# control-toolbox/CTDirect.jl

Hardware: AMD Instinct MI355X
Metric: NLP callback evals/s (constraints+sparse Jac), N-step Goddard, 1/2/4/8 GPU (higher is better)
Workload: dtype f64

## Files before the change

ctdirect.jl_amd/csrc/ctd_engine.hip:

```cpp
#include <hip/hip_runtime.h>
#include <hip/hiprtc.h>
#include <dlfcn.h>

#include <cstdio>
#include <functional>
#include <map>
#include <mutex>
#include <cstdlib>
#include <cstring>
#include <memory>
#include <new>
#include <string>
#include <vector>

#include "../../include/ctdirect_hip.h"
#include "ctd_host.hpp"
#include "ctd_kernels.hpp"
#include "ctd_hess_kernels.hpp"
#include "ctd_hess_step.hpp"
#include "ctd_iter_kernels.hpp"
#include "ctd_prod_kernels.hpp"
#include "ctd_hprod_kernels.hpp"
#include "ctd_kkt_kernels.hpp"
#include "ctd_diag_kernels.hpp"
// ... 383 lines not shown
    if (blocks > 0x7fffffff) return fail(h, CTD_EINVAL, std::string(c.fn()) + ": grid too large");
    pp.nblocks = (int32_t)blocks;
    const int32_t st = partial.grow(h, blocks * kMaxNV, c.fn());
    if (st) return st;
    pp.partial = partial.p;
    hipError_t e = hipErrorInvalidValue;
    if (h->rt) {
        const JitModule& jm = h->jit[c.op.fam][c.shard()];
        void* args[] = {&a, &x_dev};
        e = jit_launch(jm.f[c.op.f0], (int)blocks, 256, 0, h->stream, args);
        if (e == hipSuccess) e = jit_launch(jm.f[c.op.f0 + 1], 1, 64, 0, h->stream, args);
    }
    for_problem(h->model.problem, [&](auto tag) {
        using P = typename decltype(tag)::type;
        e = c.shard() ? launch_prod_units<P, K, true>(a, x_dev, h->stream) : launch_prod_units<P, K, false>(a, x_dev, h->stream);
    });
    return c.launched(h, e);
}

extern "C" {

const char* ctd_strerror(int32_t st) {
    switch (st) {
        case CTD_OK: return "ok";
        case CTD_EINVAL: return "invalid argument";
        case CTD_EGRID: return "given time grid is not strictly increasing";
        case CTD_ESCHEME: return "unknown discretization method";
        case CTD_EPATTERN: return "sparsity pattern not available";
        case CTD_EPROBLEM: return "problem not in the compiled registry";
        case CTD_ENODEVICE: return "no HIP device bound to this handle (there is no CPU fallback)";
        case CTD_EHIP: return "HIP runtime error";
        case CTD_ENOMEM: return "out of memory";
        default: return "unknown status";
    }
}

const char* ctd_last_error(const ctd_handle* h) { return h ? h->err.c_str() : g_create_err.c_str(); }

int32_t ctd_create(const ctd_desc* desc, ctd_handle** out) {
    if (!desc || !out) return fail(nullptr, CTD_EINVAL, "ctd_create: null argument");
    *out = nullptr;
    struct Del { void operator()(ctd_handle* p) const { if (p) destroy_handle(p); } };
    std::unique_ptr<ctd_handle, Del> h(new (std::nothrow) ctd_handle());
    if (!h) return fail(nullptr, CTD_ENOMEM, "ctd_create: out of memory");
    HostDesc hd{desc->problem, desc->scheme, desc->pattern_mode, desc->grid_size, desc->time_grid, desc->time_grid_len,
                desc->control_steps > 1 ? desc->control_steps : 1, desc->value_order};
    if (desc->reserved0 != 0) return fail(nullptr, CTD_EINVAL, "ctd_create: ctd_desc.reserved0 must be 0 (zero-initialise the descriptor: memset / ctd_desc d = {0})");
    std::string err;
    int st;
    try {
        st = build_model(hd, h->model, err);
    } catch (const std::bad_alloc&) {
        return fail(nullptr, CTD_ENOMEM, "ctd_create: out of memory while building the model");
    }
    if (st) return fail(nullptr, st, err);
    const Model& mo = h->model;
    if (!runtime_ocp(mo.problem)) {
        const char* bad = nullptr;
        for_problem(mo.problem, [&](auto tag) {
            using P = typename decltype(tag)::type;
            for_scheme<true>(mo.L, [&](auto t) { bad = static_layout_mismatch<P, t.sc, t.s>(mo.L); });
        });
        if (bad) return fail(nullptr, CTD_EINVAL, std::string("ctd_create: the static layout of the kernel instantiation differs from the model's layout in field '") + bad + "'");
        if (mo.pattern_mode == 0 && mo.order == 0) {
            for_problem(mo.problem, [&](auto tag) {
                using P = typename decltype(tag)::type;
                for_scheme<true>(mo.L, [&](auto t) { bad = static_emit_mismatch<P, t.sc, t.s>(mo.L, mo.Lseg, mo.vr); });
            });
            if (bad) return fail(nullptr, CTD_EINVAL, std::string("ctd_create: the static emit geometry of the kernel instantiation differs from the model's in '") + bad + "'");
        }
    }
    if (mo.L.cs > 3 && desc->device >= 0 && !runtime_ocp(mo.problem))
        return fail(nullptr, CTD_EINVAL, "ctd_create: control_steps > 3 needs an OCP registered at run time (ctd_register_ocp); the compiled registry holds the midpoint kernels for 1, 2 and 3 controls per step");
    h->step_begin = desc->step_begin;
    h->step_end = desc->step_end;
    if (h->step_begin == 0 && h->step_end == 0) h->step_end = mo.L.N;
    if (h->step_begin < 0 || h->step_end > mo.L.N || h->step_begin >= h->step_end)
        return fail(nullptr, CTD_EINVAL, "ctd_create: shard [step_begin, step_end) is not inside [0, N)");
    h->tile = env_int("CTD_TILE", 0);
    h->lean_ok = env_int("CTD_LEAN", 1) ? 1 : 0;
    if (h->lean_ok && env_int("CTD_STATIC_EMIT", 1) && !runtime_ocp(mo.problem) && mo.pattern_mode == 0 && mo.order == 0 &&
        h->step_begin == 0 && h->step_end == mo.L.N)
        h->lean_ok |= 2;
    if (h->tile <= 0) h->tile = default_tile(mo, h->step_end - h->step_begin);
    int maxb = 256;
    for_problem(mo.problem, [&](auto tag) { maxb = decltype(tag)::type::MAXB; });
    h->rt = runtime_ocp(mo.problem);
    if (h->rt) maxb = h->rt->maxb;
    h->block = env_int("CTD_BLOCK", 0);
    if (h->block <= 0) {
        h->block = 256;
        const int64_t ntl = (h->step_end - h->step_begin + h->tile - 1) / h->tile;
        if (ntl <= 512 && mo.nch_dyn <= 1 && mo.Lseg > 0 && 320 / mo.Lseg > 256 / mo.Lseg && mo.Lseg * (320 / mo.Lseg) * 10 >= 320 * 9) h->block = 320;
    }
    if (h->block < 64 || (h->block % 64)) h->block = 256;
    if (h->block > maxb) h->block = maxb;
    mo.fill_kparams(h->kp, h->step_begin, h->step_end, h->tile);
    h->lds_bytes = (size_t)lds_doubles(h->kp) * sizeof(double);
    const int debug_stop = env_int("CTD_DEBUG_STOP", 0);
    const size_t lds_cap = h->rt ? 64 * 1024 : 80 * 1024;
    while (h->lds_bytes > lds_cap && h->tile > 1) {
        h->tile = (h->tile + 1) / 2;
        mo.fill_kparams(h->kp, h->step_begin, h->step_end, h->tile);
        h->lds_bytes = (size_t)lds_doubles(h->kp) * sizeof(double);
    }
    const bool long_mid = mo.L.sc == SC_MIDPOINT && mo.L.cs == 1;
    if (desc->device >= 0 && !h->rt && env_int("CTD_TILE", 0) <= 0 && mo.nch_dyn <= 1 && (mo.L.sc == SC_IRK || long_mid) && h->tile >= 16) {
        DeviceGuard dgq(desc->device);
        if (dgq.err == hipSuccess) {
            auto resident = [&](int tile, size_t& lds) {
                KParams kq;
                mo.fill_kparams(kq, h->step_begin, h->step_end, tile);
                lds = (size_t)lds_doubles(kq) * sizeof(double);
                int r = 0;
                for_problem(mo.problem, [&](auto tag) { r = occupancy_cons_jac<typename decltype(tag)::type>(kq, h->block, lds); });
                (void)hipGetLastError();
                return r;
            };
            size_t l0 = 0;
            const int r0 = resident(h->tile, l0);
            const int64_t ns = h->step_end - h->step_begin, cap = 256 * (int64_t)r0;
            if (r0 > 0 && (ns + h->tile - 1) / h->tile >= env_int("CTD_LONG_GRID_ROUNDS", 8) * cap && maxb >= 512 && env_int("CTD_BLOCK", 0) <= 0 &&
                env_int("CTD_LONG_GRID", 1)) {
                int tbest = h->tile;
                for (int tt = h->tile + 1; tt <= 256; ++tt) {
                    KParams kq;
                    mo.fill_kparams(kq, h->step_begin, h->step_end, tt);
                    if ((size_t)lds_doubles(kq) * sizeof(double) > (long_mid ? 74u : 64u) * 1024) break;
                    tbest = tt;
                }
                if (tbest > h->tile) {
                    h->tile = tbest;
                    h->block = 512;
                    mo.fill_kparams(h->kp, h->step_begin, h->step_end, h->tile);
                    h->lds_bytes = (size_t)lds_doubles(h->kp) * sizeof(double);
                }
            } else if (mo.L.sc == SC_IRK && r0 > 0 && (ns + h->tile - 1) / h->tile > cap) {
                int tmax = 48;
                for (; tmax > h->tile; --tmax) { size_t l = 0; if (resident(tmax, l) >= r0 && l <= lds_cap) break; }
                const int64_t rounds = (ns + (int64_t)tmax * cap - 1) / ((int64_t)tmax * cap);
                const int64_t tb = (ns + rounds * cap - 1) / (rounds * cap);
                if (tb > h->tile && tb <= tmax) {
                    h->tile = (int)tb;
                    mo.fill_kparams(h->kp, h->step_begin, h->step_end, h->tile);
                    h->lds_bytes = (size_t)lds_doubles(h->kp) * sizeof(double);
                }
            }
        }
    }
    h->grid = h->kp.ntiles + h->kp.has_edge;
    h->kp.debug_stop = debug_stop;
    h->out_mb = 8.0 * ((double)(h->step_end - h->step_begin) * (mo.L.cb + mo.Lseg + (double)mo.L.nv * mo.vr)) / 1.0e6;
    h->kp.wt_store = h->out_mb <= kWtMB ? 1 : 0;
    if (const int wt = env_int("CTD_WT_STORE", -1); wt >= 0) h->kp.wt_store = wt ? 1 : 0;
    h->device = desc->device;
    if (h->device >= 0) {
        int ndev = 0;
        if (hipGetDeviceCount(&ndev) != hipSuccess || h->device >= ndev)
            return fail(nullptr, CTD_ENODEVICE, "ctd_create: HIP device not available");
        ctd_handle* hp = h.get();
        if (h->lds_bytes > 160 * 1024) return fail(nullptr, CTD_EINVAL, "ctd_create: tile does not fit the 160 KiB LDS");
        DeviceGuard dg_(hp->device); HIP_TRY(nullptr, dg_.err);
        if (desc->stream_mode == CTD_STREAM_GIVEN) { hp->stream = (hipStream_t)desc->stream; hp->own_stream = false; }
        else { HIP_TRY(nullptr, hipStreamCreateWithFlags(&hp->stream, hipStreamNonBlocking)); hp->own_stream = true; }
        HIP_TRY(nullptr, upload(hp->d_tau, mo.tau));
        HIP_TRY(nullptr, upload(hp->d_tmpl, mo.tmpl));
// ... 1740 lines not shown
```

ctdirect.jl_amd/csrc/ctd_kernel_body.hpp:

```cpp
#pragma once
#include "ctd_layout.hpp"


namespace ctd {

#if defined(CTD_SUBSTAMPS) && defined(__HIP_DEVICE_COMPILE__)
#ifndef CTD_SUB_WAVE0
#define CTD_SUB_WAVE0 0
#endif
#define CTD_SUB(kp, id)                                                                                              \
    do {                                                                                                             \
        __builtin_amdgcn_sched_barrier(0);                                                                           \
        __builtin_amdgcn_s_waitcnt(0);                                                                               \
        if ((kp).stamps && (threadIdx.x & 63) == 0 && threadIdx.x >= 64 * CTD_SUB_WAVE0 && threadIdx.x < 64 * CTD_SUB_WAVE0 + 128) \
            (kp).stamps[(size_t)gridDim.x * 12 + ((size_t)blockIdx.x * 2 + (threadIdx.x >> 6) - CTD_SUB_WAVE0) * 8 + (id)] = clock64(); \
        __builtin_amdgcn_sched_barrier(0);                                                                           \
    } while (0)
#else
#define CTD_SUB(kp, id) do { } while (0)
#endif
#if defined(CTD_SUBSTAMPS_EMIT) && defined(__HIP_DEVICE_COMPILE__)
#define CTD_SUBE(kp, id)                                                                                             \
    do {                                                                                                             \
        __builtin_amdgcn_sched_barrier(0);                                                                           \
// ... 1522 lines not shown
                        for (int u = 0; u < 4; ++u) {
                            const int s = s0 + u * par;
                            if (s < nreg) emit_store(&out[s * Ls + k], a[u] * b[u] + beta, kp.wt_store);
                        }
                    }
                }
            } else {
                uint32_t code = (hp && tid < Ls) ? pre_->b : (tid < Ls ? cx.codes[tid] : 0u);
                int q = 0;
                for (int k = tid; k < Ls; k += nthr, ++q) {
                    uint32_t nxt = 0u;
                    bool have = false;
                    if constexpr (NB > 1) {
                        if (hp && q < NB - 1) {
                            have = true;
#pragma unroll
                            for (int e = 0; e < NB - 1; ++e)
                                if (e == q) nxt = pre_->more[e];
                        }
                    }
                    if (!have) nxt = k + nthr < Ls ? cx.codes[k + nthr] : 0u;
                    const int bt = code_beta(code);
                    const double beta = bt == 0 ? 0.0 : (bt == 1 ? 1.0 : -1.0);
                    const double* pc = cx.rec + (sl0 - code_crec(code)) * stride + R.oC + code_ci(code);
                    const double* pd = cx.rec + (sl0 - code_drec(code)) * stride + code_di(code);
                    const int last = nreg - 1;
                    for (int s0 = 0; s0 < nreg; s0 += 4) {
                        double a[4], b[4];
#pragma unroll
                        for (int u = 0; u < 4; ++u) {
                            const int s = s0 + u < last ? s0 + u : last;
                            a[u] = pc[s * stride];
                            b[u] = pd[s * stride];
                        }
#pragma unroll
                        for (int u = 0; u < 4; ++u)
                            if (s0 + u < nreg) emit_store(&out[(s0 + u) * Ls + k], a[u] * b[u] + beta, kp.wt_store);
                    }
                    code = nxt;
                }
            }
        }
    }
    CTD_SUBE(kp, 2);
    if (kp.vr > 0) {
        const int vr = kp.vr;
        const int par = (int)fast_div((uint32_t)nthr, kp.div_vr);
#pragma unroll
        for (int kk = 0; kk < P::NV; ++kk) {
            double* out = out_vals<B>(kp, bl) + kp.vcol_base[kk] + cx.a * (int64_t)vr;
            const uint32_t* codes = cx.vcodes + kk * vr;
            if (par >= 1) {
                if (tid < par * vr) {
                    const int g = (int)fast_div((uint32_t)tid, kp.div_vr), k = tid - g * vr;
                    const uint32_t code = hp ? pre_->v[kk] : codes[k];
                    const double* pc = cx.rec + (slot0 + g) * stride + R.oC + code_ci(code);
                    const double* pd = cx.rec + (slot0 + g) * stride + code_di(code);
                    const int adv = par * stride;
                    if (LEAN || k >= kp.vr_early)
                        for (int s = g; s < nsteps; s += par, pc += adv, pd += adv) emit_store(&out[s * vr + k], (*pc) * (*pd), kp.wt_store);
                }
            } else {
                for (int k = tid; k < vr; k += nthr) {
                    const uint32_t code = codes[k];
                    const double* pc = cx.rec + slot0 * stride + R.oC + code_ci(code);
                    const double* pd = cx.rec + slot0 * stride + code_di(code);
                    for (int s = 0; s < nsteps; ++s, pc += stride, pd += stride) emit_store(&out[s * vr + k], (*pc) * (*pd), kp.wt_store);
                }
            }
        }
    }
    CTD_SUBE(kp, 3);
}
template <class P, int SC, int S, int NB = 1, bool B = false, bool LEAN = false>
CTD_HD void phase_emit(const KParams& kp, const BlockCtx& cx, int tid, int nthr, const EmitPreT<NB>* pre = nullptr,
                       const BatchLd bl = BatchLd{}) {
    if (pre != nullptr) phase_emit_impl<P, SC, S, NB, B, LEAN>(kp, cx, tid, nthr, *pre, pre->have != 0, bl);
    else phase_emit_impl<P, SC, S, NB, B, LEAN>(kp, cx, tid, nthr, EmitPreT<NB>{}, false, bl);
}

}

#include "ctd_emit_static.hpp"

#if !defined(__HIPCC_RTC__)
#include "ctd_problems.hpp"
#include "ctd_sym_registry.hpp"
#endif
```

ctdirect.jl_amd/csrc/ctd_kernels.hpp:

```cpp
#pragma once
#if !defined(__HIPCC_RTC__)
#include <hip/hip_runtime.h>
#include <hip/hip_ext.h>
#endif

#include "ctd_kernel_body.hpp"
#if !defined(__HIPCC_RTC__)
#include "ctd_problems.hpp"
#endif

namespace ctd {

#ifndef CTD_MULTI_TILE_LOOP
#define CTD_MULTI_TILE_LOOP 0
#endif
constexpr bool kMultiTileLoop = CTD_MULTI_TILE_LOOP != 0;

template <bool DBG>
__device__ __forceinline__ void ctd_stamp(const KParams& kp, int slot) {
    if constexpr (DBG) {
        if (kp.stamps && threadIdx.x == 0) {
            unsigned long long* p = kp.stamps + ((size_t)blockIdx.x * 6 + slot) * 2;
            p[0] = wall_clock64();
            p[1] = clock64();
// ... 42 lines not shown
template <class P, int SC, int S, bool DBG, bool B = false, bool LEAN = false>
__device__ __forceinline__ void cons_jac_body(const KParams& kp, const double* __restrict__ xu, int block, double* ctd_lds,
                                              const BatchLd bl = BatchLd{}) {
    if constexpr (B) xu += batch_member() * bl.ldx;
    ctd_pin_kernargs<SC == SC_IRK ? S : 0, LEAN>(kp, xu);
    ctd_stamp<DBG>(kp, 0);
    if (DBG && kp.debug_stop == 1) return;
    const int tid = (int)threadIdx.x, nthr = (int)blockDim.x;
    if constexpr (DirectTile<P, SC>::value) {
        const BlockCtx cx = make_direct_ctx<LEAN>(kp, block, ctd_lds, xu, LV<P, SC, S, LEAN>::blk(kp), LEAN ? P::NV : -1);
        const EmitPre pre = emit_prefetch<P, 1, LEAN>(kp, cx, tid, nthr);
        ctd_stamp<DBG>(kp, 1);
        phase_eval<P, SC, S, RegEval<P, SC, S>::value, 1, B, LEAN>(kp, cx, tid, nthr, &pre, bl);
        ctd_pin_emit_kernargs<LEAN>(kp);
        __syncthreads();
        ctd_stamp<DBG>(kp, 2);
        ctd_stamp<DBG>(kp, 3);
        if (DBG && kp.debug_stop >= 2 && kp.debug_stop <= 4) return;
        phase_emit<P, SC, S, 1, B, LEAN>(kp, cx, tid, nthr, &pre, bl);
        ctd_stamp<DBG>(kp, 4);
        if (DBG && kp.stamps) {
            __builtin_amdgcn_s_waitcnt(0);
            __syncthreads();
            ctd_stamp<DBG>(kp, 5);
        }
        return;
    }
    BlockCtx cx = make_ctx<LEAN>(kp, block, ctd_lds);
    constexpr int NB = EmitN<P, SC, S>::value;
    EmitPreT<NB> pre = {};
    const bool use_pre = !cx.is_edge && !codes_staged(kp);
    if (use_pre) pre = emit_prefetch<P, NB, LEAN>(kp, cx, tid, nthr);
    phase_load<P, SC, S, true, LEAN>(kp, cx, xu, tid, nthr);
    const int nblk = kp.ntiles + kp.has_edge;
    for (;;) {
        __syncthreads();
        ctd_stamp<DBG>(kp, 1);
        if (DBG && kp.debug_stop == 2) return;
        phase_eval<P, SC, S, false, 1, B, LEAN>(kp, cx, tid, nthr, nullptr, bl);
        ctd_pin_emit_kernargs<LEAN>(kp);
        __syncthreads();
        ctd_stamp<DBG>(kp, 2);
        if (DBG && kp.debug_stop == 3) return;
        if (!Dirs<P>::FUSED && !fin_folded<P, SC, S>(cx)) {
            phase_fin<P, SC, S>(kp, cx, tid, nthr);
            __syncthreads();
        }
        if (SC == SC_TRAPEZE) {
            phase_fin2<P, SC, S>(kp, cx, tid, nthr);
            __syncthreads();
        }
        ctd_stamp<DBG>(kp, 3);
        if (DBG && kp.debug_stop == 4) return;
        block += kp.wg_stride;
        const bool more = kMultiTileLoop && kp.wg_stride > 0 && !cx.is_edge && block < nblk;
        BlockCtx nx = cx;
        TileIn tin{0.0, 0.0, 0.0};
        if (more) {
            nx = make_ctx<LEAN>(kp, block, ctd_lds);
            tin = load_issue<P>(kp, nx, xu, tid, nthr);
        }
        phase_emit_impl<P, SC, S, NB, B, LEAN>(kp, cx, tid, nthr, pre, use_pre, bl);
        ctd_stamp<DBG>(kp, 4);
        if (!more) break;
        load_commit<P, SC, S>(kp, nx, xu, tin, tid, nthr);
        cx = nx;
    }
    if (DBG && kp.stamps) {
        __builtin_amdgcn_s_waitcnt(0);
        __syncthreads();
        ctd_stamp<DBG>(kp, 5);
    }
}

template <class P, int SC, int S> struct MinWaves {
    static constexpr int value = (P::NX <= 12 && !(SC == SC_MIDPOINT && S > 1)) ? 4 : 1;
};

template <class P, int SC, int S, bool DBG, bool LEAN = false>
__global__ void __launch_bounds__(P::MAXB, (MinWaves<P, SC, S>::value)) cons_jac_kernel(const KParams kp, const double* __restrict__ xu) {
    extern __shared__ double ctd_lds[];
    cons_jac_body<P, SC, S, DBG, false, LEAN>(kp, xu, (int)blockIdx.x, ctd_lds);
}
template <class P, int SC, int S, bool DBG, int NTHR, bool WT>
__device__ __forceinline__ void cons_jac_static_body(const KParams& kp, const double* __restrict__ xu, int block, double* ctd_lds) {
    if (__builtin_expect(block < kp.has_edge, 0)) {
        cons_jac_body<P, SC, S, DBG, false, true>(kp, xu, block, ctd_lds);
        return;
    }
#if defined(__HIP_DEVICE_COMPILE__)
    asm volatile("" ::"s"(kp.has_edge), "s"(kp.T), "s"(kp.HL), "s"(kp.HH), "s"(kp.step_begin), "s"(kp.step_end), "s"(kp.L.N),
                 "s"(kp.L.v_off), "s"(kp.L.stagewise), "s"(kp.L.euler), "s"(kp.tau), "s"(kp.L.t0), "s"(kp.L.tf), "s"(xu),
                 "s"(kp.tmpl), "s"(kp.vtmpl));
#endif
    ctd_stamp<DBG>(kp, 0);
    if (DBG && kp.debug_stop == 1) return;
    const int tid = (int)threadIdx.x;
    BlockCtx cx = make_direct_ctx<true>(kp, block, ctd_lds, xu, LV<P, SC, S, true>::blk(kp), P::NV);
    cx.is_edge = 0;
    cx.edge_part = 0;
    const EmitPre pre = emit_prefetch_static<P, SC, S, NTHR>(kp, tid);
    ctd_stamp<DBG>(kp, 1);
    phase_eval<P, SC, S, RegEval<P, SC, S>::value, 1, false, true>(kp, cx, tid, NTHR, &pre, BatchLd{});
#if defined(__HIP_DEVICE_COMPILE__)
    asm volatile("" ::"s"(kp.c), "s"(kp.vals), "s"(kp.seg_base), "s"(kp.reg_first), "s"(kp.reg_last), "s"(kp.vcol_base[0]));
#endif
    __syncthreads();
    ctd_stamp<DBG>(kp, 2);
    ctd_stamp<DBG>(kp, 3);
    if (DBG && kp.debug_stop >= 2 && kp.debug_stop <= 4) return;
    phase_emit_static<P, SC, S, NTHR, WT>(kp, cx, tid, pre);
    ctd_stamp<DBG>(kp, 4);
    if (DBG && kp.stamps) {
        __builtin_amdgcn_s_waitcnt(0);
        __syncthreads();
        ctd_stamp<DBG>(kp, 5);
    }
}
template <class P, int SC, int S, bool DBG, int NTHR, bool WT>
__global__ void __launch_bounds__(NTHR, (MinWaves<P, SC, S>::value)) cons_jac_static_kernel(const KParams kp, const double* __restrict__ xu) {
    extern __shared__ double ctd_lds[];
    cons_jac_static_body<P, SC, S, DBG, NTHR, WT>(kp, xu, (int)blockIdx.x, ctd_lds);
}
template <class P, int SC, int S>
__global__ void __launch_bounds__(P::MAXB, (MinWaves<P, SC, S>::value)) cons_jac_batch_kernel(const KParams kp, const double* __restrict__ xu,
                                                                                          const BatchLd bl) {
    extern __shared__ double ctd_lds[];
    cons_jac_body<P, SC, S, false, true>(kp, xu, (int)blockIdx.x, ctd_lds, bl);
}

struct ObjParams {
    Layout L;
    const double* tau;
    int64_t unit_begin, unit_end;
    int32_t add_mayer;
    double* partial;
    double* out;
    int32_t nblocks;
    const XHalo* halo;
    XNear near;
    int64_t ldx;
};

template <class P> __device__ double obj_time(const ObjParams& op, const double* v, int64_t i) {
    const double t0 = (P::IT0 >= 0) ? v[P::IT0 >= 0 ? P::IT0 : 0] : op.L.t0;
    const double tf = (P::ITF >= 0) ? v[P::ITF >= 0 ? P::ITF : 0] : op.L.tf;
    const double tau = op.tau ? op.tau[i] : (double)i / (double)op.L.N;
    return t0 + tau * (tf - t0);
}

template <class P, int SC>
__device__ double lagrange_unit(const ObjParams& op, const double* __restrict__ xu, const double* v, int64_t i) {
    constexpr int n = P::NX, m = P::NU;
    const Layout& L = op.L;
    const double* base = xu + i * (int64_t)L.blk;
    const int64_t gn = (i + 1) * (int64_t)L.blk;
    const double* nxt = ((op.halo && i + 1 >= op.unit_end) ? xnear(op.near, xu, gn) : xu) + gn;
    double x[n > 0 ? n : 1], u[m > 0 ? m : 1];
    if (SC == SC_TRAPEZE) {
        double w;
        if (i == 0) w = (obj_time<P>(op, v, 1) - obj_time<P>(op, v, 0)) / 2.0;
        else if (i == L.N) w = (obj_time<P>(op, v, L.N) - obj_time<P>(op, v, L.N - 1)) / 2.0;
        else w = (obj_time<P>(op, v, i + 1) - obj_time<P>(op, v, i - 1)) / 2.0;
        for (int c = 0; c < n; ++c) x[c] = base[c];
        for (int c = 0; c < m; ++c) u[c] = base[n + c];
        return w * P::template lagrange<double>(obj_time<P>(op, v, i), x, u, v);
    }
    const double ti = obj_time<P>(op, v, i), tip1 = obj_time<P>(op, v, i + 1);
    const double h = tip1 - ti;
    if (SC == SC_MIDPOINT) {
        if (L.cs > 1) {
            const double hi = h / (double)L.cs;
            for (int c = 0; c < n; ++c) x[c] = 0.5 * (base[c] + nxt[c]);
            double val = 0.0;
            for (int j = 1; j <= L.cs; ++j) {
                for (int c = 0; c < m; ++c) u[c] = base[n + (j - 1) * m + c];
                const double term = hi * P::template lagrange<double>(ti + ((double)j - 0.5) * hi, x, u, v);
                val = (j == 1) ? term : val + term;
            }
            return val;
        }
        for (int c = 0; c < m; ++c) u[c] = base[n + c];
        if (L.euler == 0) {
            for (int c = 0; c < n; ++c) x[c] = 0.5 * (base[c] + nxt[c]);
            return h * P::template lagrange<double>(0.5 * (ti + tip1), x, u, v);
        }
        for (int c = 0; c < n; ++c) x[c] = (L.euler == 1) ? base[c] : nxt[c];
        return h * P::template lagrange<double>(L.euler == 1 ? ti : tip1, x, u, v);
    }
    const double* K = base + n + L.cu;
    double local = 0.0;
    for (int j = 0; j < L.s; ++j) {
        for (int c = 0; c < n; ++c) {
            double xc = base[c];
            for (int l = 0; l < L.s; ++l) xc = xc + h * L.a[3 * j + l] * K[l * n + c];
            x[c] = xc;
        }
        const double* U = base + n + (L.stagewise ? j * m : 0);
        for (int c = 0; c < m; ++c) u[c] = U[c];
        const double term = L.b[j] * P::template lagrange<double>(ti + L.c[j] * h, x, u, v);
        local = (j == 0) ? term : local + term;
    }
    return h * local;
}

// ... 317 lines not shown
        double a = gv[k];
        for (int off = 32; off > 0; off >>= 1) a += __shfl_down(a, off, 64);
        if (lane == 0) wsum[wave][k] = a;
    }
    __syncthreads();
    if (threadIdx.x == 0)
        for (int k = 0; k < nv; ++k) {
            double sacc = 0.0;
            for (int w = 0; w < (int)(blockDim.x >> 6); ++w) sacc += wsum[w][k];
            gp.partial[((size_t)mb * gp.nblocks + block) * kMaxNV + k] = sacc;
        }
}
template <class P, int SC, int S>
__global__ void __launch_bounds__(256) __attribute__((amdgpu_waves_per_eu(2))) grad_units_kernel(const GradParams gp, const double* __restrict__ xu) {
    __shared__ double wsum[4][kMaxNV];
    const int64_t mb = batch_member();
    grad_units_body<P, SC, S>(gp, xu + mb * gp.ldx, (int)blockIdx.x, wsum, mb);
}

template <class P>
__device__ __forceinline__ void grad_finish_body(const GradParams& gp, const double* __restrict__ xu, int64_t mb = 0) {
    if (threadIdx.x >= 64) return;
    constexpr int n = P::NX, nv = P::NV;
    const Layout& L = gp.L;
    const double* part = gp.partial + (size_t)mb * gp.nblocks * kMaxNV;
    double* const g = gp.g + mb * gp.ldg;
    double gvs[nv > 0 ? nv : 1];
    for (int k = 0; k < nv; ++k) {
        double sacc = 0.0;
        for (int b = threadIdx.x; b < gp.nblocks; b += 64) sacc += part[(size_t)b * kMaxNV + k];
        for (int off = 32; off > 0; off >>= 1) sacc += __shfl_down(sacc, off, 64);
        gvs[k] = sacc;
    }
    if (threadIdx.x != 0) return;
    if (P::HAS_MAYER && (gp.owns_first || gp.owns_last)) {
        double x0[n > 0 ? n : 1], xf[n > 0 ? n : 1], v[nv > 0 ? nv : 1], g0x[n > 0 ? n : 1], gfx[n > 0 ? n : 1], gmv[nv > 0 ? nv : 1];
        const double* b0 = grad_block(gp, xu, 0);
        const double* bf = grad_block(gp, xu, L.N);
        for (int c = 0; c < n; ++c) { x0[c] = b0[c]; xf[c] = bf[c]; g0x[c] = 0.0; gfx[c] = 0.0; }
        for (int k = 0; k < nv; ++k) { v[k] = xu[L.v_off + k]; gmv[k] = 0.0; }
        mayer_partials<P, 0>(x0, xf, v, g0x, gfx, gmv);
        for (int c = 0; c < n; ++c) {
            if (gp.owns_first) g[c] += g0x[c];
            if (gp.owns_last) g[L.N * (int64_t)L.blk + c] += gfx[c];
        }
        if (gp.owns_last) for (int k = 0; k < nv; ++k) gvs[k] += gmv[k];
    }
    for (int k = 0; k < nv; ++k) g[L.v_off + k] = gvs[k];
}
template <class P>
__global__ void grad_finish_kernel(const GradParams gp, const double* __restrict__ xu) {
    if (blockIdx.x != 0) return;
    const int64_t mb = batch_member();
    grad_finish_body<P>(gp, xu + mb * gp.ldx, mb);
}

#if !defined(__HIPCC_RTC__)
template <class P>
hipError_t launch_grad(const GradParams& gp, const double* xu, int grid, hipStream_t st, int batch) {
    const dim3 g(grid > 0 ? grid : 1, batch);
    if (grid > 0)
        for_scheme<false>(gp.L, [&](auto t) { grad_units_kernel<P, t.sc, t.s><<<g, 256, 0, st>>>(gp, xu); });
    grad_finish_kernel<P><<<dim3(1, batch), 64, 0, st>>>(gp, xu);
    return hipGetLastError();
}

#endif

#if !defined(__HIPCC_RTC__)
template <class P, int SC, int S, bool DBG, bool LEAN>
hipError_t launch_variant_dbg(const KParams& kp, const double* xu, int grid, int block, size_t lds_bytes, hipStream_t st,
                              hipEvent_t e0, hipEvent_t e1) {
    if (lds_bytes > 64 * 1024) {
        hipError_t e = hipFuncSetAttribute((const void*)cons_jac_kernel<P, SC, S, DBG, LEAN>, hipFuncAttributeMaxDynamicSharedMemorySize,
                                           (int)lds_bytes);
        if (e != hipSuccess) return e;
    }
    if (e0 || e1) hipExtLaunchKernelGGL((cons_jac_kernel<P, SC, S, DBG, LEAN>), dim3(grid), dim3(block), lds_bytes, st, e0, e1, 0, kp, xu);
    else cons_jac_kernel<P, SC, S, DBG, LEAN><<<grid, block, lds_bytes, st>>>(kp, xu);
    return hipGetLastError();
}
template <class P, int SC, int S, int NTHR>
hipError_t launch_static(const KParams& kp, const double* xu, int grid, size_t lds_bytes, hipStream_t st, hipEvent_t e0, hipEvent_t e1,
                         bool dbg, bool& done) {
    done = false;
    if constexpr (StaticEmit<P, SC, S>::template built<NTHR>()) {
        using SE = StaticEmit<P, SC, S>;
        if (kp.Lseg != SE::Lseg || kp.vr != SE::vr || (SC == SC_IRK && S >= 2 && !kp.L.stagewise)) return hipSuccess;
        done = true;
        auto go = [&](auto kern) -> hipError_t {
            if (lds_bytes > 64 * 1024) {
                hipError_t e = hipFuncSetAttribute((const void*)kern, hipFuncAttributeMaxDynamicSharedMemorySize, (int)lds_bytes);
                if (e != hipSuccess) return e;
            }
            if (e0 || e1) hipExtLaunchKernelGGL(kern, dim3(grid), dim3(NTHR), lds_bytes, st, e0, e1, 0, kp, xu);
            else kern<<<grid, NTHR, lds_bytes, st>>>(kp, xu);
            return hipGetLastError();
        };
        if (dbg) return kp.wt_store ? go(cons_jac_static_kernel<P, SC, S, true, NTHR, true>) : go(cons_jac_static_kernel<P, SC, S, true, NTHR, false>);
        return kp.wt_store ? go(cons_jac_static_kernel<P, SC, S, false, NTHR, true>) : go(cons_jac_static_kernel<P, SC, S, false, NTHR, false>);
    }
    return hipSuccess;
}
template <class P, int SC, int S>
hipError_t launch_variant(const KParams& kp, const double* xu, int grid, int block, size_t lds_bytes, hipStream_t st,
                          hipEvent_t e0, hipEvent_t e1, int lean_ok) {
    const bool dbg = kp.stamps || kp.debug_stop;
    if ((lean_ok & 3) == 3 && kp.halo == nullptr && kp.n_early == 0 && (block == 256 || block == 320)) {
        bool done = false;
        const hipError_t e = block == 256 ? launch_static<P, SC, S, 256>(kp, xu, grid, lds_bytes, st, e0, e1, dbg, done)
                                          : launch_static<P, SC, S, 320>(kp, xu, grid, lds_bytes, st, e0, e1, dbg, done);
        if (done) return e;
    }
    lean_ok &= 1;
    constexpr bool kHasLean = DirectTile<P, SC>::value || SC == SC_IRK;
    if constexpr (kHasLean) {
        if (lean_ok && kp.halo == nullptr && kp.n_early == 0) {
            if (dbg) return launch_variant_dbg<P, SC, S, true, true>(kp, xu, grid, block, lds_bytes, st, e0, e1);
            return launch_variant_dbg<P, SC, S, false, true>(kp, xu, grid, block, lds_bytes, st, e0, e1);
        }
    }
    if (dbg) return launch_variant_dbg<P, SC, S, true, false>(kp, xu, grid, block, lds_bytes, st, e0, e1);
    return launch_variant_dbg<P, SC, S, false, false>(kp, xu, grid, block, lds_bytes, st, e0, e1);
}

template <class P>
hipError_t launch_cons_jac(const KParams& kp, const double* xu, int grid, int block, size_t lds_bytes, hipStream_t st,
                           hipEvent_t e0, hipEvent_t e1, int lean_ok) {
    hipError_t e = hipErrorInvalidValue;
    for_scheme<true>(kp.L, [&](auto t) { e = launch_variant<P, t.sc, t.s>(kp, xu, grid, block, lds_bytes, st, e0, e1, lean_ok); });
    return e;
}

template <class P, int SC, int S>
int occupancy_variant(int block, size_t lds_bytes) {
    int nb = 0;
    if (lds_bytes > 64 * 1024 &&
        hipFuncSetAttribute((const void*)cons_jac_kernel<P, SC, S, false>, hipFuncAttributeMaxDynamicSharedMemorySize, (int)lds_bytes) != hipSuccess)
        return 0;
    if (hipOccupancyMaxActiveBlocksPerMultiprocessor(&nb, cons_jac_kernel<P, SC, S, false>, block, lds_bytes) != hipSuccess) return 0;
    return nb;
}
template <class P, int SC, int S>
hipError_t launch_variant_batch(const KParams& kp, const double* xu, const BatchLd& bl, int grid, int block, size_t lds_bytes, hipStream_t st,
                                int batch) {
    if (lds_bytes > 64 * 1024) {
        hipError_t e = hipFuncSetAttribute((const void*)cons_jac_batch_kernel<P, SC, S>, hipFuncAttributeMaxDynamicSharedMemorySize, (int)lds_bytes);
        if (e != hipSuccess) return e;
    }
    cons_jac_batch_kernel<P, SC, S><<<dim3(grid, batch), block, lds_bytes, st>>>(kp, xu, bl);
    return hipGetLastError();
}
template <class P>
hipError_t launch_cons_jac_batch(const KParams& kp, const double* xu, const BatchLd& bl, int grid, int block, size_t lds_bytes,
                                 hipStream_t st, int batch) {
    hipError_t e = hipErrorInvalidValue;
    for_scheme<true>(kp.L, [&](auto t) { e = launch_variant_batch<P, t.sc, t.s>(kp, xu, bl, grid, block, lds_bytes, st, batch); });
    return e;
}

template <class P>
int occupancy_cons_jac(const KParams& kp, int block, size_t lds_bytes) {
    int nb = 0;
    for_scheme<true>(kp.L, [&](auto t) { nb = occupancy_variant<P, t.sc, t.s>(block, lds_bytes); });
    return nb;
}

template <class P>
hipError_t launch_obj(const ObjParams& op, const double* xu, int grid, int block, hipStream_t st, int batch) {
    const dim3 g(grid > 0 ? grid : 1, batch);
    if (grid > 0)
        for_scheme<false>(op.L, [&](auto t) { obj_partial_kernel<P, t.sc><<<g, block, 0, st>>>(op, xu); });
    obj_finish_kernel<P><<<dim3(1, batch), 64, 0, st>>>(op, xu);
    return hipGetLastError();
}

#define CTD_INSTANTIATE_LAUNCHERS(P)                                                                                       \
    template hipError_t launch_cons_jac<P>(const KParams&, const double*, int, int, size_t, hipStream_t, hipEvent_t, \
                                           hipEvent_t, int);                                                                 \
    template hipError_t launch_cons_jac_batch<P>(const KParams&, const double*, const BatchLd&, int, int, size_t, hipStream_t, int); \
    template hipError_t launch_obj<P>(const ObjParams&, const double*, int, int, hipStream_t, int);                  \
    template int occupancy_cons_jac<P>(const KParams&, int, size_t);                                                 \
    template hipError_t launch_grad<P>(const GradParams&, const double*, int, hipStream_t, int);
#define CTD_EXTERN_LAUNCHERS(P)                                                                                            \
    extern template hipError_t launch_cons_jac<P>(const KParams&, const double*, int, int, size_t, hipStream_t,      \
                                                  hipEvent_t, hipEvent_t, int);                                              \
    extern template hipError_t launch_cons_jac_batch<P>(const KParams&, const double*, const BatchLd&, int, int, size_t, hipStream_t, \
                                                        int);                                                                      \
    extern template hipError_t launch_obj<P>(const ObjParams&, const double*, int, int, hipStream_t, int);          \
    extern template int occupancy_cons_jac<P>(const KParams&, int, size_t);                                         \
    extern template hipError_t launch_grad<P>(const GradParams&, const double*, int, hipStream_t, int);

#endif

// ... 2 lines not shown
```

profiles/resource_usage.py:

```python
import argparse
import os
import re
import subprocess
from concurrent.futures import ThreadPoolExecutor

ROOT = os.path.dirname(os.path.dirname(os.path.abspath(__file__)))
CSRC = os.path.join(ROOT, "ctdirect.jl_amd", "csrc")
HIPCC = os.environ.get("HIPCC", "/opt/rocm/bin/hipcc")
KERNELS = ("jprod_kernel", "jtprod_units_kernel", "jtprod_finish_kernel", "hprod_units_kernel", "hprod_finish_kernel")
PRODUCTS = [(p, p) for p in ("quadrotor", "quadrotor12", "goddard_all", "double_integrator_free_t0_tf", "goddard",
                             "double_integrator_path", "estimate_initial_condition", "estimate_rotation_rate",
                             "least_squares_constraint", "stagewise_scalar")]
HPROD = [("double_integrator_free_t0_tf", "double_integrator_freet0tf"), ("double_integrator_path", "double_integrator_path"),
         ("estimate_initial_condition", "estimate_initial_condition"), ("estimate_rotation_rate", "estimate_rotation_rate"),
         ("goddard", "goddard"), ("goddard_all", "goddard_all"), ("least_squares_constraint", "least_squares_with_constraint"),
         ("quadrotor", "quadrotor"), ("quadrotor12", "quadrotor12"), ("stagewise_scalar", "stagewise_scalar")]
DIAG_KERNELS = ("hdiag_units_kernel", "hdiag_finish_kernel", "jsq_cols_units_kernel", "jsq_cols_finish_kernel", "jsq_rows_kernel")
SCHEMES = ("trapeze", "midpoint / Euler", "Gauss-Legendre 1", "Gauss-Legendre 2", "Gauss-Legendre 3")
FIELDS = (("vgpr", r" VGPRs: (\d+)"), ("agpr", r"AGPRs: (\d+)"), ("scratch", r"ScratchSize \[bytes/lane\]: (\d+)"),
          ("waves", r"Occupancy \[waves/SIMD\]: (\d+)"))


def remarks(stem, prefix="ctd_pkern_", kernels=KERNELS):
    r = subprocess.run([HIPCC, "--offload-arch=gfx950", "-O3", "-std=c++17", "-ffp-contract=off", "--cuda-device-only",
# ... 52 lines not shown
                assert k["scratch"] == 0 and k["shard"] == shard, (name, k)
            assert all(len(by[kn]) == 5 for kn in ("hdiag_units_kernel", "jsq_cols_units_kernel", "jsq_rows_kernel")), name
            forms.append(by)
        for i, sch in enumerate(SCHEMES):
            for by, tag in zip(forms, ("", ", shard")):
                lines.append(f"| {name} | {sch}{tag} | {cell(by['hdiag_units_kernel'][i])} | {cell(by['jsq_cols_units_kernel'][i])} | "
                             f"{cell(by['jsq_rows_kernel'][i])} |\n")
        for by, tag in zip(forms, ("", ", shard")):
            lines.append(f"| {name} | finish{tag} | {cell(by['hdiag_finish_kernel'][0])} | {cell(by['jsq_cols_finish_kernel'][0])} | | | |\n")
    with open(path, "w") as f:
        f.write(head)
        f.writelines(lines)
    print(path, len(lines) - 2, "rows")


CONS_JAC = (("cfg2", "goddard", "GoddardOCP", 2, 2, 320), ("cfg3", "double_integrator_path", "DoubleIntegratorPathOCP", 1, 1, 256),
            ("cfg4", "goddard", "GoddardOCP", 2, 3, 256))


def cons_jac_counts(stem):
    r = subprocess.run([HIPCC, "--offload-arch=gfx950", "-O3", "-std=c++17", "-ffp-contract=off", "--cuda-device-only", "-S",
                        "-Rpass-analysis=kernel-resource-usage", f"ctd_kern_{stem}.hip", "-o", "-"], cwd=CSRC, capture_output=True, text=True)
    if r.returncode:
        raise SystemExit(r.stderr[-4000:])
    res, cur = {}, None
    pats = (("sgpr", r"TotalSGPRs: (\d+)"), ("vgpr", r" VGPRs: (\d+)"), ("scratch", r"ScratchSize \[bytes/lane\]: (\d+)"),
            ("waves", r"Occupancy \[waves/SIMD\]: (\d+)"), ("sgpr_spill", r"SGPRs Spill: (\d+)"), ("vgpr_spill", r"VGPRs Spill: (\d+)"))
    for line in r.stderr.splitlines():
        m = re.search(r"Function Name: (\S+)", line)
        if m:
            cur = res.setdefault(m.group(1), {})
            continue
        if cur is not None:
            for key, pat in pats:
                m = re.search(pat, line)
                if m:
                    cur[key] = int(m.group(1))
    name, body = None, []
    for line in r.stdout.splitlines():
        m = re.match(r"^(_ZN3ctd\w*cons_jac\w*):", line)
        if m:
            name, body = m.group(1), []
            continue
        if name is None:
            continue
        m = re.search(r"; codeLenInByte = (\d+)", line)
        if m and name in res:
            ins = [l.split()[0] for l in body if l.startswith("\t") and (l.lstrip().startswith(";;#ASMSTART") or not l.lstrip().startswith((".", ";")))]
            b0 = next((i for i, x in enumerate(ins) if x == "s_barrier"), None)
            sec = []
            if b0 is not None:
                e0 = next((i for i in range(b0, len(ins)) if ins[i] in ("s_endpgm", ";;#ASMSTART")), len(ins))
                sec = ins[b0 + 1:e0]
                if e0 < len(ins) and ins[e0] == ";;#ASMSTART":
                    hi = max((i for i, x in enumerate(sec) if x.startswith("s_load")), default=-1)
                    lo, i, gap = hi, hi - 1, 0
                    while i >= 0 and gap <= 3:
                        if sec[i].startswith("s_load"):
                            lo, gap = i, 0
                        else:
                            gap += 1
                        i -= 1
                    if hi >= 0 and len(sec) - hi <= 4:
                        sec = sec[:lo]
            ins = [x for x in ins if x != ";;#ASMSTART"]
            res[name].update(code_bytes=int(m.group(1)), instructions=len(ins), sec_instructions=len(sec),
                             sec_branches=sum(x.startswith(("s_branch", "s_cbranch")) for x in sec),
                             sec_scalar_loads=sum(x.startswith("s_load") for x in sec),
                             sec_stores=sum(x.startswith("global_store") for x in sec))
            name = None
            continue
        body.append(line)
    return res


def cons_jac_table():
    print("| workload | kernel | code bytes | instructions | behind the barrier: instructions | branches | scalar loads | stores "
          "| SGPRs | VGPRs | SGPR / VGPR spills | scratch | waves/SIMD |")
    print("|---|---|---|---|---|---|---|---|---|---|---|---|---|")
    cache = {}
    for cfg, stem, ocp, sc, s, lanes in CONS_JAC:
        res = cache.setdefault(stem, cons_jac_counts(stem))
        tag = f"{len(ocp)}{ocp}ELi{sc}ELi{s}E"
        for label, suffix in (("lean", f"cons_jac_kernelINS_{tag}Lb0ELb1EEE"), (f"static, {lanes} lanes, write-through", f"cons_jac_static_kernelINS_{tag}Lb0ELi{lanes}ELb1EEE")):
            k = [v for n, v in res.items() if suffix in n]
            if not k:
                print(f"| {cfg} | {label} | not built |")
                continue
            k = k[0]
            assert k["scratch"] == 0, (cfg, label, k)
            print(f"| {cfg} | {label} | {k['code_bytes']} | {k['instructions']} | {k['sec_instructions']} | {k['sec_branches']} | {k['sec_scalar_loads']} "
                  f"| {k['sec_stores']} | {k['sgpr']} | {k['vgpr']} | {k['sgpr_spill']} / {k['vgpr_spill']} | {k['scratch']} | {k['waves']} |")


KRYLOV_KERNELS = ("krylov_init_kernel", "krylov_first_kernel", "krylov_alfa_kernel", "krylov_lanczos_kernel", "krylov_update_kernel")


def krylov_table():
    ks = remarks("ctd_krylov", "", KRYLOV_KERNELS)
    assert [k["kernel"] for k in ks] == list(KRYLOV_KERNELS), ks
    path = os.path.join(ROOT, "profiles", "kkt_minres_resources.md")
    lines = ["# Resources of the MINRES vector kernels (csrc/ctd_krylov.hip)\n\n",
             "From the compiler's remarks for gfx950 (`python profiles/resource_usage.py --krylov`, no GPU needed).  The kernels do not\n"
             "depend on the OCP: one instantiation each.  The script fails if any of them uses scratch.\n\n",
             "| kernel | VGPR + AGPR | scratch B/lane | waves/SIMD |\n", "|---|---|---|---|\n"]
    for k in ks:
        assert k["scratch"] == 0, k
        lines.append(f"| {k['kernel']} | {k['vgpr']} + {k['agpr']} | {k['scratch']} | {k['waves']} |\n")
    with open(path, "w") as f:
        f.writelines(lines)
    print(path, len(ks), "kernels")


def main():
    ap = argparse.ArgumentParser()
    ap.add_argument("--jobs", type=int, default=8)
    ap.add_argument("--krylov", action="store_true", help="write profiles/kkt_minres_resources.md (the MINRES vector kernels) and stop")
    ap.add_argument("--cons-jac", action="store_true", help="print the table of profiles/static_emit.md (lean and static-emit kernels of cfg2 / cfg3 / cfg4) and stop")
    args = ap.parse_args()
    if args.cons_jac:
        return cons_jac_table()
    if args.krylov:
        return krylov_table()
    stems = [s for s, _ in PRODUCTS]
    with ThreadPoolExecutor(args.jobs) as ex:
        table = dict(zip(stems, ex.map(remarks, stems)))
    write("products_resource_usage.log", PRODUCTS, table, False)
    write("hprod_resource_usage.log", HPROD, table, True)
    with ThreadPoolExecutor(args.jobs) as ex:
        dtable = dict(zip(stems, ex.map(lambda s: remarks(s, "ctd_dkern_", DIAG_KERNELS), stems)))
        stable = dict(zip(stems, ex.map(lambda s: remarks(s, "ctd_dskern_", DIAG_KERNELS), stems)))
    write_diag(dtable, stable)


if __name__ == "__main__":
    main()
```

Before: 187,800.

## Add static role-per-thread evaluation phase to static cons/jac kernel

Adds a compile-time specialised evaluation phase for the static-emit constraint/Jacobian kernel. Threads are assigned fixed roles (dynamics stage, path constraint, lead finalisation) times slot index, with wave-uniform range checks so whole waves skip roles they do not own. It is enabled by default through a new lean_ok bit and replaces the generic phase_eval when the role count fits the block. It also hoists more kernel parameters into SGPRs before the edge branch. In exchange it doubles the number of static kernel instantiations and may raise register pressure; it applies only to IRK schemes with one dynamics chunk.

```diff
diff --git a/ctdirect.jl_amd/csrc/ctd_engine.hip b/ctdirect.jl_amd/csrc/ctd_engine.hip
--- a/ctdirect.jl_amd/csrc/ctd_engine.hip
+++ b/ctdirect.jl_amd/csrc/ctd_engine.hip
@@ -489,6 +489,7 @@
     if (h->lean_ok && env_int("CTD_STATIC_EMIT", 1) && !runtime_ocp(mo.problem) && mo.pattern_mode == 0 && mo.order == 0 &&
         h->step_begin == 0 && h->step_end == mo.L.N)
         h->lean_ok |= 2;
+    if ((h->lean_ok & 2) && env_int("CTD_STATIC_EVAL", 1)) h->lean_ok |= 4;
     if (h->tile <= 0) h->tile = default_tile(mo, h->step_end - h->step_begin);
     int maxb = 256;
     for_problem(mo.problem, [&](auto tag) { maxb = decltype(tag)::type::MAXB; });
diff --git a/ctdirect.jl_amd/csrc/ctd_eval_static.hpp b/ctdirect.jl_amd/csrc/ctd_eval_static.hpp
--- /dev/null
+++ b/ctdirect.jl_amd/csrc/ctd_eval_static.hpp
@@ -0,0 +1,63 @@
+#pragma once
+
+namespace ctd {
+
+template <class P, int SC, int S> struct StaticEval {
+    static constexpr int r_dyn = StagePoints<SC, S>::value * Dirs<P>::NCH_DYN;
+    static constexpr int r_path = (P::NPATH > 0) ? Dirs<P>::NCH_PATH : 0;
+    static constexpr int roles = r_dyn + r_path + 1;
+    static constexpr bool offered = Dirs<P>::FUSED && DirectTile<P, SC>::value && SC == SC_IRK && Dirs<P>::NCH_DYN == 1;
+};
+CTD_HD int static_eval_lg(int ns) { return ns <= 1 ? 0 : 32 - __builtin_clz((unsigned)(ns - 1)); }
+template <class P, int SC, int S, int NTHR> CTD_HD bool static_eval_fits(int ns) {
+    return StaticEval<P, SC, S>::offered && (StaticEval<P, SC, S>::roles << static_eval_lg(ns)) <= NTHR;
+}
+
+template <class P, int SC, int S, int NTHR>
+CTD_HD void phase_eval_static(const KParams& kp, const BlockCtx& cx, int tid) {
+    using SE = StaticEval<P, SC, S>;
+    constexpr RecLayout R = RL<P, SC, S>::R;
+    constexpr bool REG = RegEval<P, SC, S>::value;
+    constexpr int lead = SE::r_dyn + SE::r_path;
+    const int ns = cx.nslots;
+    const int lg = static_eval_lg(ns);
+    const int k = tid & ((1 << lg) - 1), role = tid >> lg;
+#if defined(__HIP_DEVICE_COMPILE__)
+    const int w0 = __builtin_amdgcn_readfirstlane(tid) & ~63;
+#else
+    const int w0 = tid & ~63;
+#endif
+    const int rlo = w0 >> lg, rhi = (w0 + 63) >> lg;
+    if (rlo < SE::r_dyn) {
+        if (role < SE::r_dyn && k < ns) {
+            const int j = role;
+            double* ev = cx.rec + k * R.stride + R.oEval + j * R.eval_sz;
+            if constexpr (REG) {
+                double evr[R.eval_sz];
+#pragma unroll
+                for (int e = 0; e < R.eval_sz; ++e) evr[e] = 0.0;
+                eval_dynamics<P, SC, S, false, true>(kp, cx, k, j, 0, evr);
+                fin_stage<P, SC, S, true>(kp, cx, k, j, evr);
+                const int64_t i = slot_index<true>(kp, cx, k);
+                if (i >= 0 && i < kp.L.N) {
+#pragma unroll
+                    for (int e = 0; e < R.eval_sz; ++e) ev[e] = evr[e];
+                }
+            } else {
+                eval_dynamics<P, SC, S, false, true>(kp, cx, k, j, 0, ev);
+                fin_stage<P, SC, S, true>(kp, cx, k, j, ev);
+            }
+        }
+    }
+    if constexpr (SE::r_path > 0) {
+        if (rlo < lead && rhi >= SE::r_dyn) {
+            if (role >= SE::r_dyn && role < lead && k < ns) eval_step_path<P, SC, S, REG, true>(kp, cx, k, role - SE::r_dyn);
+        }
+    }
+    if (rlo <= lead && rhi >= lead) {
+        if (role == lead && k < ns) fin_lead<P, SC, S, true>(kp, cx, k);
+    }
+    if (tid < ns) cx.rec[tid * R.stride] = 1.0;
+}
+
+}
diff --git a/ctdirect.jl_amd/csrc/ctd_kernel_body.hpp b/ctdirect.jl_amd/csrc/ctd_kernel_body.hpp
--- a/ctdirect.jl_amd/csrc/ctd_kernel_body.hpp
+++ b/ctdirect.jl_amd/csrc/ctd_kernel_body.hpp
@@ -1628,6 +1628,7 @@
 }
 
 #include "ctd_emit_static.hpp"
+#include "ctd_eval_static.hpp"
 
 #if !defined(__HIPCC_RTC__)
 #include "ctd_problems.hpp"
diff --git a/ctdirect.jl_amd/csrc/ctd_kernels.hpp b/ctdirect.jl_amd/csrc/ctd_kernels.hpp
--- a/ctdirect.jl_amd/csrc/ctd_kernels.hpp
+++ b/ctdirect.jl_amd/csrc/ctd_kernels.hpp
@@ -148,17 +148,27 @@
     extern __shared__ double ctd_lds[];
     cons_jac_body<P, SC, S, DBG, false, LEAN>(kp, xu, (int)blockIdx.x, ctd_lds);
 }
-template <class P, int SC, int S, bool DBG, int NTHR, bool WT>
+template <class P, int SC, int S, bool DBG, int NTHR, bool WT, bool SEV>
 __device__ __forceinline__ void cons_jac_static_body(const KParams& kp, const double* __restrict__ xu, int block, double* ctd_lds) {
+    if constexpr (SEV) {
+#if defined(__HIP_DEVICE_COMPILE__)
+        asm volatile("" ::"s"(kp.has_edge), "s"(kp.T), "s"(kp.HL), "s"(kp.HH), "s"(kp.ntiles), "s"(kp.step_begin), "s"(kp.step_end),
+                     "s"(kp.L.N), "s"(kp.L.v_off), "s"(kp.L.stagewise), "s"(kp.L.euler), "s"(kp.tau), "s"(kp.L.t0), "s"(kp.L.tf), "s"(xu),
+                     "s"(kp.tmpl), "s"(kp.vtmpl), "s"(kp.stage_codes), "s"(kp.Lseg), "s"(kp.vr), "s"(kp.c), "s"(kp.vals), "s"(kp.seg_base),
+                     "s"(kp.reg_first), "s"(kp.reg_last), "s"(kp.vcol_base[0]));
+#endif
+    }
     if (__builtin_expect(block < kp.has_edge, 0)) {
         cons_jac_body<P, SC, S, DBG, false, true>(kp, xu, block, ctd_lds);
         return;
     }
+    if constexpr (!SEV) {
 #if defined(__HIP_DEVICE_COMPILE__)
-    asm volatile("" ::"s"(kp.has_edge), "s"(kp.T), "s"(kp.HL), "s"(kp.HH), "s"(kp.step_begin), "s"(kp.step_end), "s"(kp.L.N),
-                 "s"(kp.L.v_off), "s"(kp.L.stagewise), "s"(kp.L.euler), "s"(kp.tau), "s"(kp.L.t0), "s"(kp.L.tf), "s"(xu),
-                 "s"(kp.tmpl), "s"(kp.vtmpl));
-#endif
+        asm volatile("" ::"s"(kp.has_edge), "s"(kp.T), "s"(kp.HL), "s"(kp.HH), "s"(kp.step_begin), "s"(kp.step_end), "s"(kp.L.N),
+                     "s"(kp.L.v_off), "s"(kp.L.stagewise), "s"(kp.L.euler), "s"(kp.tau), "s"(kp.L.t0), "s"(kp.L.tf), "s"(xu),
+                     "s"(kp.tmpl), "s"(kp.vtmpl));
+#endif
+    }
     ctd_stamp<DBG>(kp, 0);
     if (DBG && kp.debug_stop == 1) return;
     const int tid = (int)threadIdx.x;
@@ -167,7 +177,8 @@
     cx.edge_part = 0;
     const EmitPre pre = emit_prefetch_static<P, SC, S, NTHR>(kp, tid);
     ctd_stamp<DBG>(kp, 1);
-    phase_eval<P, SC, S, RegEval<P, SC, S>::value, 1, false, true>(kp, cx, tid, NTHR, &pre, BatchLd{});
+    if (SEV && __builtin_expect(static_eval_fits<P, SC, S, NTHR>(cx.nslots), 1)) phase_eval_static<P, SC, S, NTHR>(kp, cx, tid);
+    else phase_eval<P, SC, S, RegEval<P, SC, S>::value, 1, false, true>(kp, cx, tid, NTHR, &pre, BatchLd{});
 #if defined(__HIP_DEVICE_COMPILE__)
     asm volatile("" ::"s"(kp.c), "s"(kp.vals), "s"(kp.seg_base), "s"(kp.reg_first), "s"(kp.reg_last), "s"(kp.vcol_base[0]));
 #endif
@@ -183,10 +194,10 @@
         ctd_stamp<DBG>(kp, 5);
     }
 }
-template <class P, int SC, int S, bool DBG, int NTHR, bool WT>
+template <class P, int SC, int S, bool DBG, int NTHR, bool WT, bool SEV>
 __global__ void __launch_bounds__(NTHR, (MinWaves<P, SC, S>::value)) cons_jac_static_kernel(const KParams kp, const double* __restrict__ xu) {
     extern __shared__ double ctd_lds[];
-    cons_jac_static_body<P, SC, S, DBG, NTHR, WT>(kp, xu, (int)blockIdx.x, ctd_lds);
+    cons_jac_static_body<P, SC, S, DBG, NTHR, WT, SEV>(kp, xu, (int)blockIdx.x, ctd_lds);
 }
 template <class P, int SC, int S>
 __global__ void __launch_bounds__(P::MAXB, (MinWaves<P, SC, S>::value)) cons_jac_batch_kernel(const KParams kp, const double* __restrict__ xu,
@@ -670,7 +681,7 @@
 }
 template <class P, int SC, int S, int NTHR>
 hipError_t launch_static(const KParams& kp, const double* xu, int grid, size_t lds_bytes, hipStream_t st, hipEvent_t e0, hipEvent_t e1,
-                         bool dbg, bool& done) {
+                         bool dbg, bool sev, bool& done) {
     done = false;
     if constexpr (StaticEmit<P, SC, S>::template built<NTHR>()) {
         using SE = StaticEmit<P, SC, S>;
@@ -685,8 +696,12 @@
             else kern<<<grid, NTHR, lds_bytes, st>>>(kp, xu);
             return hipGetLastError();
         };
-        if (dbg) return kp.wt_store ? go(cons_jac_static_kernel<P, SC, S, true, NTHR, true>) : go(cons_jac_static_kernel<P, SC, S, true, NTHR, false>);
-        return kp.wt_store ? go(cons_jac_static_kernel<P, SC, S, false, NTHR, true>) : go(cons_jac_static_kernel<P, SC, S, false, NTHR, false>);
+        auto pick = [&](auto sv) -> hipError_t {
+            constexpr bool SEV = decltype(sv)::value;
+            if (dbg) return kp.wt_store ? go(cons_jac_static_kernel<P, SC, S, true, NTHR, true, SEV>) : go(cons_jac_static_kernel<P, SC, S, true, NTHR, false, SEV>);
+            return kp.wt_store ? go(cons_jac_static_kernel<P, SC, S, false, NTHR, true, SEV>) : go(cons_jac_static_kernel<P, SC, S, false, NTHR, false, SEV>);
+        };
+        return sev ? pick(std::true_type{}) : pick(std::false_type{});
     }
     return hipSuccess;
 }
@@ -696,8 +711,9 @@
     const bool dbg = kp.stamps || kp.debug_stop;
     if ((lean_ok & 3) == 3 && kp.halo == nullptr && kp.n_early == 0 && (block == 256 || block == 320)) {
         bool done = false;
-        const hipError_t e = block == 256 ? launch_static<P, SC, S, 256>(kp, xu, grid, lds_bytes, st, e0, e1, dbg, done)
-                                          : launch_static<P, SC, S, 320>(kp, xu, grid, lds_bytes, st, e0, e1, dbg, done);
+        const bool sev = (lean_ok & 4) != 0;
+        const hipError_t e = block == 256 ? launch_static<P, SC, S, 256>(kp, xu, grid, lds_bytes, st, e0, e1, dbg, sev, done)
+                                          : launch_static<P, SC, S, 320>(kp, xu, grid, lds_bytes, st, e0, e1, dbg, sev, done);
         if (done) return e;
     }
     lean_ok &= 1;
diff --git a/profiles/resource_usage.py b/profiles/resource_usage.py
--- a/profiles/resource_usage.py
+++ b/profiles/resource_usage.py
@@ -158,7 +158,9 @@
     for cfg, stem, ocp, sc, s, lanes in CONS_JAC:
         res = cache.setdefault(stem, cons_jac_counts(stem))
         tag = f"{len(ocp)}{ocp}ELi{sc}ELi{s}E"
-        for label, suffix in (("lean", f"cons_jac_kernelINS_{tag}Lb0ELb1EEE"), (f"static, {lanes} lanes, write-through", f"cons_jac_static_kernelINS_{tag}Lb0ELi{lanes}ELb1EEE")):
+        for label, suffix in (("lean", f"cons_jac_kernelINS_{tag}Lb0ELb1EEE"),
+                              (f"static, {lanes} lanes, write-through, generic evaluation", f"cons_jac_static_kernelINS_{tag}Lb0ELi{lanes}ELb1ELb0EEE"),
+                              (f"static, {lanes} lanes, write-through, static evaluation", f"cons_jac_static_kernelINS_{tag}Lb0ELi{lanes}ELb1ELb1EEE")):
             k = [v for n, v in res.items() if suffix in n]
             if not k:
                 print(f"| {cfg} | {label} | not built |")
```

Result: slower. 131,000 (-30.2%).
